# FueledByRedBull/audio-forge

Measured on AMD Instinct MI355X. Metric: 48 kHz mono frames/s (real-time-factor x streams), voice chain, higher is better.
Workload: dtype f64

## Files before the change

### audio-forge_amd/csrc/af_rnnoise.hip

```cpp
#include <hip/hip_runtime.h>
#include <cstdlib>

#include "af_dsp.h"
#include "af_fft_consts.h"
#include "af_suppressor.h"
#include "af_switches.hpp"

namespace af {

__constant__ int c_eband[kRnnBands] = {0, 1, 2, 3, 4, 5, 6, 7, 8, 10, 12, 14, 16, 20, 24, 28, 34, 40, 48, 60, 78, 100};

__constant__ uint16_t c_blk_first[54] = {0, 4, 8, 12, 16, 20, 24, 28, 32, 40, 48, 56, 64, 72, 80, 88, 96, 104, 112, 120, 128, 136, 144, 152, 160, 168, 176, 184, 192, 200, 208, 216, 224, 232, 240, 248, 256, 264, 272, 280, 288, 296, 304, 312, 320, 328, 336, 344, 352, 360, 368, 376, 384, 392};
__constant__ uint8_t c_blk_count[54] = {4, 4, 4, 4, 4, 4, 4, 4, 8, 8, 8, 8, 8, 8, 8, 8, 8, 8, 8, 8, 8, 8, 8, 8, 8, 8, 8, 8, 8, 8, 8, 8, 8, 8, 8, 8, 8, 8, 8, 8, 8, 8, 8, 8, 8, 8, 8, 8, 8, 8, 8, 8, 8, 8};
__constant__ uint8_t c_seg_blk0[21] = {0, 1, 2, 3, 4, 5, 6, 7, 8, 9, 10, 11, 12, 14, 16, 18, 21, 24, 28, 34, 43};
__constant__ uint8_t c_seg_nblk[21] = {1, 1, 1, 1, 1, 1, 1, 1, 1, 1, 1, 1, 2, 2, 2, 3, 3, 4, 6, 9, 11};
constexpr int kBandBlocks = 54;
constexpr int kFftBuf = 15 * 72;
constexpr int kFftWaves = 4;
#ifndef AF_FFT_PREFETCH
#define AF_FFT_PREFETCH 1
#endif
constexpr int kBandSkewLen = 404 + (404 >> 3) + 1;

__device__ __forceinline__ int band_skew(int bin) { return bin + (bin >> 3); }

struct FftShared {
  float2 tw960[15 * 64];
  float2 tw64[8 * 8];
  float win[kRnnFrame];
  float frac[kBandSkewLen];
  int32_t band_of[484];
  float dct6[kRnnBands * 6];
  uint16_t blk_first[64];
  uint8_t blk_count[64], seg_blk0[32], seg_nblk[32];
};

__device__ __forceinline__ float2 cmul(float2 x, float2 w) { return make_float2(x.x * w.x - x.y * w.y, x.x * w.y + x.y * w.x); }
__device__ __forceinline__ float2 cadd(float2 x, float2 y) { return make_float2(x.x + y.x, x.y + y.y); }
__device__ __forceinline__ float2 csub(float2 x, float2 y) { return make_float2(x.x - y.x, x.y - y.y); }
__device__ __forceinline__ float2 mulmj(float2 z) { return make_float2(z.y, -z.x); }

__device__ __forceinline__ void wave_lds_fence() {
  __asm__ volatile("s_waitcnt lgkmcnt(0)" ::: "memory");
  __builtin_amdgcn_wave_barrier();
}

__device__ __forceinline__ void dft3(float2 x0, float2 x1, float2 x2, float2 &y0, float2 &y1, float2 &y2) {
  const float c = 0.86602540378443864676f;
  const float2 t = cadd(x1, x2), d = csub(x1, x2);
  y0 = cadd(x0, t);
  const float2 m = make_float2(x0.x - 0.5f * t.x, x0.y - 0.5f * t.y);
  const float2 sj = make_float2(d.y * c, -d.x * c);
  y1 = cadd(m, sj);
  y2 = csub(m, sj);
}
__device__ __forceinline__ void dft5(const float2 *x, float2 *y) {
  const float c1 = 0.30901699437494742410f, c2 = -0.80901699437494742410f;
  const float s1 = 0.95105651629515357212f, s2 = 0.58778525229247312917f;
  const float2 t1 = cadd(x[1], x[4]), t2 = cadd(x[2], x[3]), d1 = csub(x[1], x[4]), d2 = csub(x[2], x[3]);
  y[0] = make_float2(x[0].x + t1.x + t2.x, x[0].y + t1.y + t2.y);
  const float2 m1 = make_float2(x[0].x + c1 * t1.x + c2 * t2.x, x[0].y + c1 * t1.y + c2 * t2.y);
  const float2 m2 = make_float2(x[0].x + c2 * t1.x + c1 * t2.x, x[0].y + c2 * t1.y + c1 * t2.y);
  const float2 n1 = mulmj(make_float2(s1 * d1.x + s2 * d2.x, s1 * d1.y + s2 * d2.y));
  const float2 n2 = mulmj(make_float2(s2 * d1.x - s1 * d2.x, s2 * d1.y - s1 * d2.y));
  y[1] = cadd(m1, n1);
  y[4] = csub(m1, n1);
  y[2] = cadd(m2, n2);
  y[3] = csub(m2, n2);
}
__device__ __forceinline__ void dft8(const float2 *v, float2 *V) {
  const float h = 0.70710678118654752440f;
  const float2 a0 = cadd(v[0], v[4]), a1 = csub(v[0], v[4]), a2 = cadd(v[2], v[6]), a3 = mulmj(csub(v[2], v[6]));
  const float2 a4 = cadd(v[1], v[5]), a5 = csub(v[1], v[5]), a6 = cadd(v[3], v[7]), a7 = mulmj(csub(v[3], v[7]));
  const float2 b0 = cadd(a0, a2), b2 = csub(a0, a2), b1 = cadd(a1, a3), b3 = csub(a1, a3);
  const float2 b4 = cadd(a4, a6), b6 = csub(a4, a6), b5 = cadd(a5, a7), b7 = csub(a5, a7);
  const float2 w1 = make_float2((b5.x + b5.y) * h, (b5.y - b5.x) * h);
  const float2 w2 = mulmj(b6);
  const float2 w3 = make_float2((b7.y - b7.x) * h, -(b7.x + b7.y) * h);
  V[0] = cadd(b0, b4);
  V[4] = csub(b0, b4);
  V[1] = cadd(b1, w1);
  V[5] = csub(b1, w1);
  V[2] = cadd(b2, w2);
  V[6] = csub(b2, w2);
  V[3] = cadd(b3, w3);
  V[7] = csub(b3, w3);
}

__device__ __forceinline__ void fft_shared_init(FftShared &S, const SuppTables &tb, int tid, int nthreads) {
  for (int i = tid; i < 15 * 64; i += nthreads) S.tw960[i] = tb.twiddle[(i & 63) * (i >> 6)];
  for (int i = tid; i < 64; i += nthreads) S.tw64[i] = tb.twiddle[15 * (i & 7) * (i >> 3)];
  for (int i = tid; i < kRnnFrame; i += nthreads) S.win[i] = tb.half_window[i];
  for (int i = tid; i < 404; i += nthreads) S.frac[band_skew(i)] = tb.frac[i];
  for (int i = tid; i < 484; i += nthreads) S.band_of[i] = tb.band_of_bin[i];
  for (int i = tid; i < kRnnBands * 6; i += nthreads) S.dct6[i] = tb.dct[(i / 6) * kRnnBands + (i % 6)];
  if (tid < 54) {
    S.blk_first[tid] = c_blk_first[tid];
    S.blk_count[tid] = c_blk_count[tid];
  }
  if (tid < 21) {
    S.seg_blk0[tid] = c_seg_blk0[tid];
    S.seg_nblk[tid] = c_seg_nblk[tid];
  }
}

__device__ __forceinline__ void fft960_wave(float2 *a, const FftShared &S, int lane, float scale) {
  float2 x[15];
#pragma unroll
  for (int n1 = 0; n1 < 15; ++n1) x[n1] = a[64 * n1 + lane];
  wave_lds_fence();
  {
    float2 t[3][5];
#pragma unroll
    for (int nb = 0; nb < 5; ++nb)
      dft3(x[(3 * nb) % 15], x[(5 + 3 * nb) % 15], x[(10 + 3 * nb) % 15], t[0][nb], t[1][nb], t[2][nb]);
#pragma unroll
    for (int ka = 0; ka < 3; ++ka) {
      float2 y[5];
      dft5(t[ka], y);
#pragma unroll
      for (int kb = 0; kb < 5; ++kb) {
        const int k1 = (10 * ka + 6 * kb) % 15;
        a[k1 * 72 + lane] = cmul(y[kb], S.tw960[k1 * 64 + lane]);
      }
      __builtin_amdgcn_sched_barrier(0);
    }
  }
  wave_lds_fence();
  {
    const int q = lane & 7;
#pragma unroll
    for (int half = 0; half < 2; ++half) {
      const int id = lane + 64 * half, k1 = id >> 3;
      if (id < 120) {
        float2 v[8], V[8];
#pragma unroll
        for (int pp = 0; pp < 8; ++pp) v[pp] = a[k1 * 72 + 8 * pp + q];
        wave_lds_fence();
        dft8(v, V);
        a[k1 * 72 + q] = V[0];
#pragma unroll
        for (int r = 1; r < 8; ++r) a[k1 * 72 + r * 9 + q] = cmul(V[r], S.tw64[r * 8 + q]);
      }
      __builtin_amdgcn_sched_barrier(0);
    }
  }
  wave_lds_fence();
  {
    float2 v0[8], v1[8];
    const int id1 = lane + 64;
    const int k1a = lane >> 3, r = lane & 7, k1b = id1 >> 3;
#pragma unroll
    for (int q = 0; q < 8; ++q) v0[q] = a[k1a * 72 + r * 9 + q];
    if (id1 < 120) {
#pragma unroll
      for (int q = 0; q < 8; ++q) v1[q] = a[k1b * 72 + r * 9 + q];
    }
    wave_lds_fence();
    float2 V[8];
    dft8(v0, V);
#pragma unroll
    for (int t = 0; t < 8; ++t) a[k1a + 15 * (r + 8 * t)] = make_float2(V[t].x * scale, V[t].y * scale);
    if (id1 < 120) {
      dft8(v1, V);
#pragma unroll
      for (int t = 0; t < 8; ++t) a[k1b + 15 * (r + 8 * t)] = make_float2(V[t].x * scale, V[t].y * scale);
    }
  }
  wave_lds_fence();
}

template <int kBegin, int kEnd, typename F>
__device__ __forceinline__ void static_for(F &&f) {
  if constexpr (kBegin < kEnd) {
    f(std::integral_constant<int, kBegin>{});
    static_for<kBegin + 1, kEnd>(f);
  }
}
template <int kCtrl>
__device__ __forceinline__ float dpp_move(float v) {
  return __int_as_float(__builtin_amdgcn_update_dpp(__float_as_int(v), __float_as_int(v), kCtrl, 0xf, 0xf, false));
}
__device__ __forceinline__ float wave_allsum_xor(float acc) {
  {
    const auto r = __builtin_amdgcn_permlane32_swap(__float_as_uint(acc), __float_as_uint(acc), false, false);
    acc = __uint_as_float(r[0]) + __uint_as_float(r[1]);
  }
  {
    const auto r = __builtin_amdgcn_permlane16_swap(__float_as_uint(acc), __float_as_uint(acc), false, false);
    acc = __uint_as_float(r[0]) + __uint_as_float(r[1]);
  }
  acc = acc + dpp_move<0x128>(acc);
  acc = acc + dpp_move<0x124>(acc);
  acc = acc + dpp_move<0x4E>(acc);
  acc = acc + dpp_move<0xB1>(acc);
  return acc;
}
template <int kN>
__device__ __forceinline__ float wave_dot64_n(const float *x, const float *y, int lane) {
  float acc = 0.0f;
  const float *xl = x + lane, *yl = y + lane;
#pragma unroll
  for (int k = 0; k < (kN + 63) / 64; ++k) {
    if (64 * k + 63 < kN) acc = acc + xl[64 * k] * yl[64 * k];
    else if (lane < kN - 64 * k) acc = acc + xl[64 * k] * yl[64 * k];
  }
  return wave_allsum_xor(acc);
}
__device__ __forceinline__ float wave_dot64_sq_stride2(const float *y, int n, int lane) {
  float acc = 0.0f;
  for (int i = lane; i < n; i += 64) acc = acc + y[2 * i] * y[2 * i];
  return wave_allsum_xor(acc);
}

__device__ __forceinline__ float band_sums_wave(const float *prod, float *scratch, const FftShared &S, int lane) {
  wave_lds_fence();
  float rise = 0.0f, fall = 0.0f;
  if (lane < kBandBlocks) {
    const int e0 = S.blk_first[lane], count = S.blk_count[lane];
#pragma unroll
    for (int j = 0; j < 8; ++j) {
      if (j < count) {
        const int idx = band_skew(e0 + j);
        const float tmp = prod[idx];
        const float fr = S.frac[idx];
        fall += (1 - fr) * tmp;
        rise += fr * tmp;
      }
    }
  }
  scratch[lane] = rise;
  scratch[64 + lane] = fall;
  wave_lds_fence();
  float band = 0.0f;
  if (lane < kRnnBands) {
    float r = 0.0f, f = 0.0f;
    if (lane > 0) {
      const int k0 = S.seg_blk0[lane - 1], nk = S.seg_nblk[lane - 1];
      for (int k = 0; k < nk; ++k) r += scratch[k0 + k];
    }
    if (lane < kRnnBands - 1) {
      const int k0 = S.seg_blk0[lane], nk = S.seg_nblk[lane];
      for (int k = 0; k < nk; ++k) f += scratch[64 + k0 + k];
    }
    band = r + f;
    if (lane == 0 || lane == kRnnBands - 1) band *= 2;
  }
  wave_lds_fence();
  return band;
}

__device__ __forceinline__ float interp_gain(const float *bandE, const FftShared &S, int bin) {
  if (bin >= (100 << 2)) return 0.0f;
  const int b = S.band_of[bin];
  const float f = S.frac[band_skew(bin)];
  return (1 - f) * bandE[b] + f * bandE[b + 1];
}

struct FftUnitLds {
  float2 fa[kFftBuf];
  __device__ float *prod() { return reinterpret_cast<float *>(fa + kRnnFreq + 1); }
  __device__ float *scratch() { return prod() + kBandSkewLen + 1; }
  __device__ float *small() { return scratch() + 128; }
};
static_assert((kRnnFreq + 1) * 2 + kBandSkewLen + 1 + 128 + 6 * 32 <= kFftBuf * 2, "the tail of the transform buffer holds the band work arrays");


constexpr int kFramesPerWave = 10;

__device__ __forceinline__ float window_at(const FftShared &S, int i) { return S.win[i < kRnnFrame ? i : kRnnWindow - 1 - i]; }

extern "C" __global__ __launch_bounds__(64 * kFftWaves, 3) void supp_spectrum_kernel(SuppArgs a, SuppTables tb) {
  __shared__ FftShared S;
  __shared__ FftUnitLds U[kFftWaves];
  const int tid = threadIdx.x, wave = tid >> 6, lane = tid & 63;
  fft_shared_init(S, tb, tid, 64 * kFftWaves);
  __syncthreads();
  const int groups = (a.n_frames + kFramesPerWave - 1) / kFramesPerWave;
  const int64_t unit = (int64_t)blockIdx.x * kFftWaves + wave;
  if (unit >= (int64_t)a.n_streams * groups) return;
  const int s = (int)(unit / groups), fg = (int)(unit % groups);
  const int64_t n = (int64_t)a.n_frames * kRnnFrame;
  FftUnitLds &L = U[wave];
  float nxt[15];
  auto fetch = [&](int f) {
    const float *pb = a.xh + (int64_t)s * (kPitchBuf + n) + (int64_t)(f + 1) * kRnnFrame;
#pragma unroll
    for (int j = 0; j < 15; ++j) nxt[j] = pb[kPitchBuf - kRnnWindow + lane + 64 * j];
  };
  const int f_end = (fg + 1) * kFramesPerWave < a.n_frames ? (fg + 1) * kFramesPerWave : a.n_frames;
  fetch(fg * kFramesPerWave);
  for (int f = fg * kFramesPerWave; f < f_end; ++f) {
    const int64_t cell = (int64_t)f * a.n_streams + s;
#pragma unroll
    for (int j = 0; j < 15; ++j) L.fa[lane + 64 * j] = make_float2(nxt[j] * window_at(S, lane + 64 * j), 0.0f);
#if AF_FFT_PREFETCH
    if (f + 1 < f_end) fetch(f + 1);
#endif
    wave_lds_fence();
    fft960_wave(L.fa, S, lane, 1.0f / kRnnWindow);
#if !AF_FFT_PREFETCH
    if (f + 1 < f_end) fetch(f + 1);
#endif
    float2 *Xg = a.X + cell * kRnnFreq;
    float *prod = L.prod();
#pragma unroll
    for (int j = 0; j < 8; ++j) {
      const int i = lane + 64 * j;
      if (i < kRnnFreq) {
        const float2 x = L.fa[i];
        Xg[i] = x;
        if (i < 400) prod[band_skew(i)] = x.x * x.x + x.y * x.y;
      }
    }
    const float ex = band_sums_wave(prod, L.scratch(), S, lane);
    if (lane < kRnnBands) a.rec[cell].Ex[lane] = ex;
  }
}

struct PitchLds {
  float ds[kPitchBuf / 2];
  float ylk[(kPitchMax >> 1) + 4];
  float ceps[kCepsMem][kRnnBands];
  float Ex[kRnnBands], Ly[kRnnBands];
  float feat[kRnnFeatPad];
  float dist[kCepsMem][kCepsMem];
};

template <int MP>
__device__ __forceinline__ void best_pitch_scan_wave(const float *numa, const float *da, float *syy, float Syy, int lane, int &bp0, int &bp1) {
#pragma unroll 8
  for (int i = 0; i < MP; ++i) {
    syy[i] = Syy;
    Syy = fmaxf(1.0f, Syy + da[i]);
  }
  wave_lds_fence();
  float bn0 = -1, bn1 = -1, bd0 = 0, bd1 = 0;
  bp0 = 0;
  bp1 = 1;
#pragma unroll
  for (int base = 0; base < MP; base += 64) {
    const int i = base + lane;
    const float num = i < MP ? numa[i] : -1.0f;
    const float sy = i < MP ? syy[i] : 1.0f;
    unsigned long long todo = ~0ull;
    for (;;) {
      const bool pass = num >= 0.0f && num * bd1 > bn1 * sy;
      const unsigned long long m = __ballot(pass) & todo;
      if (m == 0) break;
      const int k = __ffsll((long long)m) - 1;
      const float nk = __int_as_float(__builtin_amdgcn_readlane(__float_as_int(num), k));
      const float sk = __int_as_float(__builtin_amdgcn_readlane(__float_as_int(sy), k));
      if (nk * bd0 > bn0 * sk) {
        bn1 = bn0; bd1 = bd0; bp1 = bp0;
        bn0 = nk; bd0 = sk; bp0 = base + k;
      } else {
        bn1 = nk; bd1 = sk; bp1 = base + k;
      }
      todo = k == 63 ? 0ull : ~0ull << (k + 1);
    }
  }
}

constexpr int kPsFrames = 4;
constexpr int kPsX0 = 255;
constexpr int kPsRaw = kPitchBuf + (kPsFrames - 1) * kRnnFrame;
struct PsScan {
  union {
    struct { float d4[kPitchBuf / 4]; float numa[152], da[152], syy[152]; float x4z[672]; } c;
    struct { float xc[304], numa[304], da[304], syy[304]; } f;
  };
};
struct alignas(16) PitchSearch4Lds {
  float ds[kPsFrames][kPitchBuf / 2];
  union {
    float raw[kPsRaw];
    PsScan scan[kPsFrames];
  };
};
#ifdef AF_PS_PROFILE
#define AF_PS_DECL long long ps_t[9]; ps_t[8] = clock64()
#define AF_PS_STAMP(k) ps_t[k] = clock64()
#define AF_PS_PRINT                                                                                                        \
  if (lane == 0 && wave == 0 && (blockIdx.x == 0 || blockIdx.x == gridDim.x / 2))                                          \
  printf("pitch search wg %u: span %lld | decimate %lld | autocorr+lpc %lld | whiten+store %lld | coarse xcorr %lld | coarse scan %lld | " \
         "fine xcorr %lld | fine scan %lld | total %lld cycles\n", blockIdx.x, ps_t[0] - ps_t[8], ps_t[1] - ps_t[0], ps_t[2] - ps_t[1],     \
         ps_t[3] - ps_t[2], ps_t[4] - ps_t[3], ps_t[5] - ps_t[4], ps_t[6] - ps_t[5], ps_t[7] - ps_t[6], ps_t[7] - ps_t[8])
#else
#define AF_PS_DECL
#define AF_PS_STAMP(k)
#define AF_PS_PRINT
#endif
extern "C" __global__ __launch_bounds__(64 * kPsFrames, 4) void supp_pitchsearch4_kernel(SuppArgs a, SuppTables tb) {
  __shared__ PitchSearch4Lds L;
  AF_PS_DECL;
  const int tid = threadIdx.x, wave = tid >> 6, lane = tid & 63;
  const int groups = (a.n_frames + kPsFrames - 1) / kPsFrames;
  const int s = (int)(blockIdx.x / groups), f0 = (int)(blockIdx.x % groups) * kPsFrames;
  const int f = f0 + wave;
  const bool live = f < a.n_frames;
  const int64_t n = (int64_t)a.n_frames * kRnnFrame;
  const float *xh = a.xh + (int64_t)s * (kPitchBuf + n);
  {
    const int frames_here = (a.n_frames - f0) < kPsFrames ? (a.n_frames - f0) : kPsFrames;
    const int span = kPitchBuf + (frames_here - 1) * kRnnFrame;
    const float4 *src = reinterpret_cast<const float4 *>(xh + (int64_t)(f0 + 1) * kRnnFrame);
    float4 *dst = reinterpret_cast<float4 *>(L.raw);
    for (int i = tid; i < span / 4; i += 64 * kPsFrames) dst[i] = src[i];
  }
  __syncthreads();
  AF_PS_STAMP(0);
  float *ds = L.ds[wave];
  if (live) {
    const float *pb = L.raw + wave * kRnnFrame;
    static_for<0, (kPitchBuf / 2 + 63) / 64>([&](auto r_tag) {
      constexpr int r = decltype(r_tag)::value;
      const int i = lane + 64 * r;
      if (64 * r + 63 < kPitchBuf / 2 || lane < kPitchBuf / 2 - 64 * r) {
        if (r == 0) ds[i] = i == 0 ? .5f * (.5f * pb[1] + pb[0]) : .5f * (.5f * (pb[2 * i - 1] + pb[2 * i + 1]) + pb[2 * i]);
        else ds[i] = .5f * (.5f * (pb[2 * i - 1] + pb[2 * i + 1]) + pb[2 * i]);
      }
    });
  }
  __syncthreads();
  if (!live) return;
  AF_PS_STAMP(1);
  PsScan &S = L.scan[wave];
  const int64_t cell = (int64_t)f * a.n_streams + s;
  SuppFrameRec *rec = a.rec + cell;
  float n0, n1, n2, n3, n4;
  {
    float ac[5];
    static_for<0, 5>([&](auto k_tag) {
      constexpr int k = decltype(k_tag)::value;
      ac[k] = wave_dot64_n<kPitchBuf / 2 - k>(ds + k, ds, lane);
    });
    ac[0] *= 1.0001f;
    for (int i = 1; i <= 4; ++i) ac[i] -= ac[i] * (.008f * i) * (.008f * i);
    float lpc[4] = {0, 0, 0, 0};
    float error = ac[0];
    if (ac[0] != 0) {
      for (int i = 0; i < 4; ++i) {
        float rr = 0;
        for (int j = 0; j < i; ++j) rr += lpc[j] * ac[i - j];
        rr += ac[i + 1];
        const float r = -rr / error;
        lpc[i] = r;
        for (int j = 0; j < (i + 1) >> 1; ++j) {
          const float t1 = lpc[j], t2 = lpc[i - 1 - j];
          lpc[j] = t1 + r * t2;
          lpc[i - 1 - j] = t2 + r * t1;
        }
        error = error - r * r * error;
        if (error < .001f * ac[0]) break;
      }
    }
    float tmp = 1.0f;
    for (int i = 0; i < 4; ++i) {
      tmp = .9f * tmp;
      lpc[i] = lpc[i] * tmp;
    }
    const float c1 = .8f;
    n0 = lpc[0] + .8f;
    n1 = lpc[1] + c1 * lpc[0];
    n2 = lpc[2] + c1 * lpc[1];
    n3 = lpc[3] + c1 * lpc[2];
    n4 = c1 * lpc[3];
  }
  AF_PS_STAMP(2);
  {
    constexpr int kRounds = (kPitchBuf / 2 + 63) / 64;
    float yv[kRounds];
    static_for<0, kRounds>([&](auto r_tag) {
      constexpr int r = decltype(r_tag)::value;
      const int i = lane + 64 * r;
      float sum = 0.0f;
      if (64 * r + 63 < kPitchBuf / 2 || lane < kPitchBuf / 2 - 64 * r) {
        sum = ds[i];
        if (r == 0) {
          sum += n0 * (i >= 1 ? ds[i >= 1 ? i - 1 : 0] : 0.0f);
          sum += n1 * (i >= 2 ? ds[i >= 2 ? i - 2 : 0] : 0.0f);
          sum += n2 * (i >= 3 ? ds[i >= 3 ? i - 3 : 0] : 0.0f);
          sum += n3 * (i >= 4 ? ds[i >= 4 ? i - 4 : 0] : 0.0f);
          sum += n4 * (i >= 5 ? ds[i >= 5 ? i - 5 : 0] : 0.0f);
        } else {
          sum += n0 * ds[i - 1];
          sum += n1 * ds[i - 2];
          sum += n2 * ds[i - 3];
          sum += n3 * ds[i - 4];
          sum += n4 * ds[i - 5];
        }
      }
      yv[r] = sum;
    });
    wave_lds_fence();
    float *dsg = a.ds + cell * (kPitchBuf / 2);
    static_for<0, kRounds>([&](auto r_tag) {
      constexpr int r = decltype(r_tag)::value;
      const int i = lane + 64 * r;
      if (64 * r + 63 < kPitchBuf / 2 || lane < kPitchBuf / 2 - 64 * r) {
        ds[i] = yv[r];
        dsg[i] = yv[r];
      }
    });
  }
  wave_lds_fence();
  AF_PS_STAMP(3);
  const int max_pitch = kPitchMax - 3 * kPitchMin;
  const float *x_lp = ds + (kPitchMax >> 1);
  int best0, best1;
  {
    constexpr int len = kRnnWindow >> 2, mp = (kPitchMax - 3 * kPitchMin) >> 2;
    static_assert(kPsX0 + (len - 1) + ((len - 1) >> 4) < 672 && 3 + 4 * 95 + 23 + kPsX0 < 672, "x4z holds the data and both guards");
    for (int i = lane; i < kPsX0; i += 64) S.c.x4z[i] = 0.0f;
    for (int i = kPsX0 + len + ((len - 1) >> 4) + lane; i < 672; i += 64) S.c.x4z[i] = 0.0f;
    for (int i = lane; i < kPitchBuf / 4; i += 64) {
      const float v = ds[2 * i];
      S.c.d4[i] = v;
      const int j = i - (kPitchMax >> 2);
      if (j >= 0 && j < len) S.c.x4z[kPsX0 + j + (j >> 4)] = v;
    }
    wave_lds_fence();
    {
      typedef float v4f_ps __attribute__((ext_vector_type(4)));
      v4f_ps acc = {0.0f, 0.0f, 0.0f, 0.0f};
      const int col = lane & 15, kq = lane >> 4;
      const float *ap = S.c.d4 + kq + col;
      const float *bp = S.c.x4z + kPsX0 + kq - 17 * col;
#pragma unroll
      for (int st = 0; st < 96; ++st) {
        const float av = ap[4 * st];
        const float bv = bp[4 * st + (st >> 2)];
        acc = __builtin_amdgcn_mfma_f32_16x16x4f32(av, bv, acc, 0, 0, 0);
      }
#pragma unroll
      for (int r = 0; r < 4; ++r) {
        const int lag = 16 * col + kq * 4 + r;
        if (lag < mp) {
          const float sum = acc[r];
          const float x16 = sum * 1e-12f;
          S.c.numa[lag] = sum > 0 ? x16 * x16 : -1.0f;
          const float ya = S.c.d4[lag + len], yb = S.c.d4[lag];
          S.c.da[lag] = ya * ya - yb * yb;
        }
      }
    }
    AF_PS_STAMP(4);
    float Syy0;
    {
      float acc = 0.0f;
      for (int i = lane; i < len; i += 64) acc = acc + S.c.d4[i] * S.c.d4[i];
      Syy0 = 1.0f + wave_allsum_xor(acc);
    }
    wave_lds_fence();
    static_assert(mp == 147, "coarse lag count");
    best_pitch_scan_wave<mp>(S.c.numa, S.c.da, S.c.syy, Syy0, lane, best0, best1);
  }
  AF_PS_STAMP(5);
  wave_lds_fence();
  {
    constexpr int len = kRnnWindow >> 1, mp = (kPitchMax - 3 * kPitchMin) >> 1;
    for (int i = lane; i < mp; i += 64) {
      S.f.xc[i] = 0.0f;
      S.f.numa[i] = -1.0f;
      const float ya = ds[i + len], yb = ds[i];
      S.f.da[i] = ya * ya - yb * yb;
    }
    wave_lds_fence();
    for (int c = 0; c < 2; ++c) {
      const int centre = 2 * (c == 0 ? best0 : best1);
      for (int i = centre - 2; i <= centre + 2; ++i) {
        if (i < 0 || i >= mp) continue;
        if (c == 1) {
          const int d0 = i - 2 * best0;
          if (d0 <= 2 && d0 >= -2) continue;
        }
        const float v = fmaxf(-1.0f, wave_dot64_n<len>(x_lp, ds + i, lane));
        if (lane == 0) {
          S.f.xc[i] = v;
          const float x16 = v * 1e-12f;
          S.f.numa[i] = v > 0 ? x16 * x16 : -1.0f;
        }
      }
    }
    AF_PS_STAMP(6);
    const float Syy0 = 1.0f + wave_dot64_n<len>(ds, ds, lane);
    wave_lds_fence();
    best_pitch_scan_wave<mp>(S.f.numa, S.f.da, S.f.syy, Syy0, lane, best0, best1);
  }
  int pitch_index;
  {
    int offset = 0;
    if (best0 > 0 && best0 < (max_pitch >> 1) - 1) {
      const float pa = S.f.xc[best0 - 1], pbv = S.f.xc[best0], pc = S.f.xc[best0 + 1];
      if ((pc - pa) > .7f * (pbv - pa)) offset = 1;
      else if ((pa - pc) > .7f * (pbv - pc)) offset = -1;
    }
    pitch_index = kPitchMax - (2 * best0 - offset);
  }
  if (lane == 0) rec->pitch_index = pitch_index;
  AF_PS_STAMP(7);
  AF_PS_PRINT;
}

extern "C" __global__ __launch_bounds__(64, 6) void supp_pitch_kernel(SuppArgs a, SuppTables tb) {
  __shared__ PitchLds L;
  const int lane = threadIdx.x;
  const int s = blockIdx.x;
  const int64_t n = (int64_t)a.n_frames * kRnnFrame;
  const float *xh = a.xh + (int64_t)s * (kPitchBuf + n);
  float *st = a.state + (int64_t)s * SuppState::kCount;
  int last_period = (int)st[SuppState::kLastPeriod];
  float last_gain = st[SuppState::kLastGain];
  int memid = (int)st[SuppState::kMemId];
  for (int i = lane; i < kCepsMem * kRnnBands; i += 64) (&L.ceps[0][0])[i] = st[SuppState::kCeps + i];
  __syncthreads();

  constexpr int kDsRegs = (kPitchBuf / 2 + 63) / 64;
  float ds_next[kDsRegs];
  float ex_next = 0.0f;
  int pitch_next = 0;
  auto prefetch = [&](int f) {
    const SuppFrameRec *rn = a.rec + ((int64_t)f * a.n_streams + s);
    const float *dsg = a.ds + ((int64_t)f * a.n_streams + s) * (kPitchBuf / 2);
#pragma unroll
    for (int k2 = 0; k2 < kDsRegs; ++k2) {
      const int i = lane + 64 * k2;
      ds_next[k2] = i < kPitchBuf / 2 ? dsg[i] : 0.0f;
    }
    ex_next = lane < kRnnBands ? rn->Ex[lane] : 0.0f;
    pitch_next = rn->pitch_index;
  };
  if (a.n_frames > 0) prefetch(0);
  for (int f = 0; f < a.n_frames; ++f) {
    SuppFrameRec *rec = a.rec + ((int64_t)f * a.n_streams + s);
    if (lane < kRnnBands) L.Ex[lane] = ex_next;
#pragma unroll
    for (int k2 = 0; k2 < kDsRegs; ++k2) {
      const int i = lane + 64 * k2;
      if (i < kPitchBuf / 2) L.ds[i] = ds_next[k2];
    }
    int pitch_index = __builtin_amdgcn_readfirstlane(pitch_next);
    const float ex_mine = ex_next;
    if (f + 1 < a.n_frames) prefetch(f + 1);
    __syncthreads();
    float gain;
    {
      const int minperiod0 = kPitchMin;
      const int maxperiod = kPitchMax / 2, minperiod = kPitchMin / 2, N = kRnnWindow / 2;
      int T0 = pitch_index / 2;
      const int prev_period = last_period / 2;
      const float *x = L.ds + maxperiod;
      if (T0 >= maxperiod) T0 = maxperiod - 1;
      const float xx = wave_dot64_n<N>(x, x, lane);
      float xy = wave_dot64_n<N>(x, x - T0, lane);
      {
        const int chunk = (maxperiod + 63) / 64;
        float local[6];
        float acc = 0.0f;
#pragma unroll
        for (int k2 = 0; k2 < 6; ++k2) {
          const int i = lane * chunk + k2 + 1;
          if (i <= maxperiod) acc = acc + (x[-i] * x[-i] - x[N - i] * x[N - i]);
          local[k2] = acc;
        }
        float total = acc;
#pragma unroll
        for (int off = 1; off < 64; off <<= 1) {
          const float other = __shfl_up(total, off);
          if (lane >= off) total = total + other;
        }
        const float before = __shfl_up(total, 1);
        if (lane == 0) L.ylk[0] = xx;
#pragma unroll
        for (int k2 = 0; k2 < 6; ++k2) {
          const int i = lane * chunk + k2 + 1;
          if (i <= maxperiod) L.ylk[i] = fmaxf(0.0f, xx + (lane == 0 ? local[k2] : before + local[k2]));
        }
      }
      __syncthreads();
      float yy = L.ylk[T0];
      float best_xy = xy, best_yy = yy;
      const float g0 = xy / sqrtf(1 + xx * yy);
      float g = g0;
      int T = T0;
      float xy_k[16], yy_k[16];
      int T1_k[16];
      static_for<2, 16>([&](auto k_tag) {
        constexpr int k2 = decltype(k_tag)::value;
        const int T1 = (2 * T0 + k2) / (2 * k2);
        int T1b;
        if (k2 == 2) T1b = (T1 + T0 > maxperiod) ? T0 : T0 + T1;
        else {
          constexpr int sc2 = (k2 == 6 || k2 == 12) ? 5 : ((k2 & 1) ? 2 : 3);
          T1b = (2 * sc2 * T0 + k2) / (2 * k2);
        }
        T1_k[k2] = T1;
        if (T1 >= minperiod) {
          xy_k[k2] = __int_as_float(__builtin_amdgcn_readfirstlane(
              __float_as_int(.5f * (wave_dot64_n<N>(x, x - T1, lane) + wave_dot64_n<N>(x, x - T1b, lane)))));
          yy_k[k2] = __int_as_float(__builtin_amdgcn_readfirstlane(__float_as_int(.5f * (L.ylk[T1] + L.ylk[T1b]))));
        } else {
          xy_k[k2] = 0.0f;
          yy_k[k2] = 0.0f;
        }
        if (k2 & 1) __builtin_amdgcn_sched_barrier(0);
      });
      bool past_min = false;
      static_for<2, 16>([&](auto k_tag) {
        constexpr int k2 = decltype(k_tag)::value;
        const int T1 = T1_k[k2];
        if (T1 < minperiod) past_min = true;
        if (past_min) return;
        xy = xy_k[k2];
        yy = yy_k[k2];
        const float g1 = xy / sqrtf(1 + xx * yy);
        float cont;
        const int dT = T1 - prev_period;
        if (dT <= 1 && dT >= -1) cont = last_gain;
        else if (dT <= 2 && dT >= -2 && 5 * k2 * k2 < T0) cont = .5f * last_gain;
        else cont = 0;
        float thresh = fmaxf(.3f, .7f * g0 - cont);
        if (T1 < 3 * minperiod) thresh = fmaxf(.4f, .85f * g0 - cont);
        else if (T1 < 2 * minperiod) thresh = fmaxf(.5f, .9f * g0 - cont);
        if (g1 > thresh) {
          best_xy = xy;
          best_yy = yy;
          T = T1;
          g = g1;
        }
      });
      best_xy = fmaxf(0.0f, best_xy);
      float pg = (best_yy <= best_xy) ? 1.0f : best_xy / (best_yy + 1);
      const float c0 = wave_dot64_n<N>(x, x - (T - 1), lane);
      const float c1v = wave_dot64_n<N>(x, x - T, lane);
      const float c2 = wave_dot64_n<N>(x, x - (T + 1), lane);
      int offset = 0;
      if ((c2 - c0) > .7f * (c1v - c0)) offset = 1;
      else if ((c0 - c2) > .7f * (c1v - c2)) offset = -1;
      if (pg > g) pg = g;
      pitch_index = 2 * T + offset;
      if (pitch_index < minperiod0) pitch_index = minperiod0;
      gain = pg;
    }
    last_period = pitch_index;
    last_gain = gain;
    float dctcol[kRnnBands];
    {
      int col = lane < kRnnBands ? lane : 0;
      asm volatile("" : "+v"(col));
#pragma unroll
      for (int j = 0; j < kRnnBands; ++j) dctcol[j] = tb.dct[j * kRnnBands + col];
    }
    float E = 0.0f;
    {
      const float ly_raw = log10f(1e-2f + ex_mine);
      float logMax = -2, follow = -2, ly_mine = 0.0f;
#pragma unroll
      for (int i = 0; i < kRnnBands; ++i) {
        float ly = __int_as_float(__builtin_amdgcn_readlane(__float_as_int(ly_raw), i));
        ly = fmaxf(logMax - 7, fmaxf(follow - 1.5f, ly));
        if (lane == i) ly_mine = ly;
        logMax = fmaxf(logMax, ly);
        follow = fmaxf(follow - 1.5f, ly);
        E += __int_as_float(__builtin_amdgcn_readlane(__float_as_int(ex_mine), i));
      }
      if (lane < kRnnBands) L.Ly[lane] = ly_mine;
    }
    const bool silence = E < 0.04f;
    if (lane < kRnnFeatPad) L.feat[lane] = 0.0f;
    __syncthreads();
    if (!silence) {
      if (lane == 6) L.feat[kRnnBands + 18] = .01f * (pitch_index - 300);
      if (lane < kRnnBands) {
        float sum = 0;
#pragma unroll
        for (int j = 0; j < kRnnBands; ++j) sum += L.Ly[j] * dctcol[j];
        float v = sum * sqrtf(2.0f / 22);
        if (lane == 0) v -= 12;
        if (lane == 1) v -= 4;
        L.feat[lane] = v;
        L.ceps[memid][lane] = v;
      }
      __syncthreads();
      const int m1 = memid < 1 ? kCepsMem + memid - 1 : memid - 1;
      const int m2 = memid < 2 ? kCepsMem + memid - 2 : memid - 2;
      if (lane < 6) {
        const float c0 = L.ceps[memid][lane], c1v = L.ceps[m1][lane], c2 = L.ceps[m2][lane];
        L.feat[lane] = c0 + c1v + c2;
        L.feat[kRnnBands + lane] = c0 - c2;
        L.feat[kRnnBands + 6 + lane] = c0 - 2 * c1v + c2;
      }
      memid = memid + 1 == kCepsMem ? 0 : memid + 1;
      {
        const int i = lane >> 3, j = lane & 7;
        float dist = 0;
        for (int k2 = 0; k2 < kRnnBands; ++k2) {
          const float t = L.ceps[i][k2] - L.ceps[j][k2];
          dist += t * t;
        }
        L.dist[i][j] = dist;
      }
      __syncthreads();
      {
        float mindist = 1e15f;
        if (lane < kCepsMem) {
#pragma unroll
          for (int j = 0; j < kCepsMem; ++j)
            if (j != lane) mindist = fminf(mindist, L.dist[lane][j]);
        }
        float spec_variability = 0;
#pragma unroll
        for (int i = 0; i < kCepsMem; ++i) spec_variability += __int_as_float(__builtin_amdgcn_readlane(__float_as_int(mindist), i));
        if (lane == 0) L.feat[kRnnBands + 19] = spec_variability / kCepsMem - 2.1f;
      }
    }
    __syncthreads();
    if (lane < kRnnFeatPad) rec->feat[lane] = L.feat[lane];
    if (lane == 0) {
      rec->silence = silence ? 1 : 0;
      rec->pitch_index = pitch_index;
    }
    __syncthreads();
  }
  if (lane == 0) {
    st[SuppState::kLastPeriod] = (float)last_period;
    st[SuppState::kLastGain] = last_gain;
    st[SuppState::kMemId] = (float)memid;
  }
  for (int i = lane; i < kCepsMem * kRnnBands; i += 64) st[SuppState::kCeps + i] = (&L.ceps[0][0])[i];
  for (int i = lane; i < kPitchBuf; i += 64) st[SuppState::kHist + i] = xh[n + i];
}

extern "C" __global__ __launch_bounds__(64 * kFftWaves, 3) void supp_pitchspec_kernel(SuppArgs a, SuppTables tb) {
  __shared__ FftShared S;
  __shared__ FftUnitLds U[kFftWaves];
  const int tid = threadIdx.x, wave = tid >> 6, lane = tid & 63;
  fft_shared_init(S, tb, tid, 64 * kFftWaves);
  __syncthreads();
  const int groups = (a.n_frames + kFramesPerWave - 1) / kFramesPerWave;
  const int64_t unit = (int64_t)blockIdx.x * kFftWaves + wave;
  if (unit >= (int64_t)a.n_streams * groups) return;
  const int s = (int)(unit / groups), fg = (int)(unit % groups);
  const int64_t n = (int64_t)a.n_frames * kRnnFrame;
  FftUnitLds &L = U[wave];
  const int f_begin = fg * kFramesPerWave;
  const int f_end = (fg + 1) * kFramesPerWave < a.n_frames ? (fg + 1) * kFramesPerWave : a.n_frames;
  int my_pitch = 0, my_silence = 0;
  if (f_begin + lane < f_end) {
    const SuppFrameRec *r = a.rec + ((int64_t)(f_begin + lane) * a.n_streams + s);
    my_pitch = r->pitch_index;
    my_silence = r->silence;
  }
  float nxt[15];
  auto fetch = [&](int f) {
    const int pitch_index = __builtin_amdgcn_readlane(my_pitch, f - f_begin);
    const float *pb = a.xh + (int64_t)s * (kPitchBuf + n) + (int64_t)(f + 1) * kRnnFrame;
#pragma unroll
    for (int j = 0; j < 15; ++j) nxt[j] = pb[kPitchBuf - kRnnWindow - pitch_index + lane + 64 * j];
  };
  fetch(f_begin);
  for (int f = f_begin; f < f_end; ++f) {
    const int64_t cell = (int64_t)f * a.n_streams + s;
    SuppFrameRec *rec = a.rec + cell;
    const bool silence = __builtin_amdgcn_readlane(my_silence, f - f_begin) != 0;
    const float2 *Xg = a.X + cell * kRnnFreq;
    float2 Xr[8];
#pragma unroll
    for (int j = 0; j < 8; ++j) {
      const int i = lane + 64 * j;
      Xr[j] = i < kRnnFreq ? Xg[i] : make_float2(0.0f, 0.0f);
    }
    float ex = 0.0f;
    if (lane < kRnnBands) ex = rec->Ex[lane];
#pragma unroll
    for (int j = 0; j < 15; ++j) L.fa[lane + 64 * j] = make_float2(nxt[j] * window_at(S, lane + 64 * j), 0.0f);
#if AF_FFT_PREFETCH
    if (f + 1 < f_end) fetch(f + 1);
#endif
    wave_lds_fence();
    fft960_wave(L.fa, S, lane, 1.0f / kRnnWindow);
#if !AF_FFT_PREFETCH
    if (f + 1 < f_end) fetch(f + 1);
#endif
    float2 *Pg = a.P + cell * kRnnFreq;
    float *prod = L.prod();
    float2 Pr[7];
#pragma unroll
    for (int j = 0; j < 8; ++j) {
      const int i = lane + 64 * j;
      if (i < kRnnFreq) {
        const float2 p = L.fa[i];
        Pg[i] = p;
        if (j < 7) Pr[j] = p;
        if (i < 400) prod[band_skew(i)] = p.x * p.x + p.y * p.y;
      }
    }
// ... 569 lines not shown
```

Measured before the change: 13.02 billion.

## Shrink coarse pitch MFMA to ten rows and scan fine candidates in registers

The coarse cross-correlation MFMA now runs 64 steps over a 10-row lag map instead of 96 steps over a padded layout, using a new index-map header with different LDS padding. The fine pitch search no longer fills and scans a full 304-lag array. It keeps the up to ten candidate correlations in lanes, computes the running Syy prefix only up to the highest candidate, and picks the best two with a ballot-based scan. This cuts LDS traffic and serial scan work, at the cost of more intricate index logic that must reproduce the original tie-breaking and Syy accumulation exactly.

```diff
diff --git a/audio-forge_amd/csrc/af_pitch_coarse_map.h b/audio-forge_amd/csrc/af_pitch_coarse_map.h
--- /dev/null
+++ b/audio-forge_amd/csrc/af_pitch_coarse_map.h
@@ -0,0 +1,39 @@
+#pragma once
+
+namespace af {
+namespace pitch_coarse {
+
+constexpr int kSteps = 64;
+constexpr int kLen = 240;
+constexpr int kLags = 147;
+constexpr int kRows = 10;
+constexpr int kYLen = 432;
+constexpr int kXGuardLo = 15;
+constexpr int kXGuardHi = 16;
+constexpr int kXWords = kXGuardLo + kLen + kXGuardHi;
+
+constexpr int y_word(int m) { return m + (m >> 4); }
+constexpr int kYWords = y_word(kYLen - 1) + 1;
+
+constexpr int lane_row(int lane) { return lane & 15; }
+constexpr int lane_k(int lane) { return lane >> 4; }
+constexpr int used_row(int row) { return row < kRows ? row : kRows - 1; }
+
+constexpr int y_index(int step, int k, int row) { return 4 * step + k + 16 * used_row(row); }
+constexpr int x_index(int step, int k, int col) { return 4 * step + k - col; }
+
+constexpr int a_base(int k, int row) { return 17 * used_row(row) + k; }
+constexpr int a_step(int step) { return 4 * step + (step >> 2); }
+constexpr int a_word(int step, int k, int row) { return a_base(k, row) + a_step(step); }
+constexpr int b_base(int k, int col) { return kXGuardLo + k - col; }
+constexpr int b_step(int step) { return 4 * step; }
+constexpr int b_word(int step, int k, int col) { return b_base(k, col) + b_step(step); }
+
+constexpr int out_row(int lane, int r) { return 4 * (lane >> 4) + r; }
+constexpr int out_lag(int lane, int r) { return 16 * out_row(lane, r) + (lane & 15); }
+
+static_assert(a_word(kSteps - 1, 3, kRows - 1) == y_word(4 * (kSteps - 1) + 3 + 16 * (kRows - 1)), "the padded word of the largest y index");
+static_assert(a_word(kSteps - 1, 3, 15) < kYWords && b_word(kSteps - 1, 3, 0) == kXWords - 1 && b_word(0, 0, 15) == 0, "operand ranges");
+
+}
+}
diff --git a/audio-forge_amd/csrc/af_rnnoise.hip b/audio-forge_amd/csrc/af_rnnoise.hip
--- a/audio-forge_amd/csrc/af_rnnoise.hip
+++ b/audio-forge_amd/csrc/af_rnnoise.hip
@@ -3,6 +3,7 @@
 
 #include "af_dsp.h"
 #include "af_fft_consts.h"
+#include "af_pitch_coarse_map.h"
 #include "af_suppressor.h"
 #include "af_switches.hpp"
 
@@ -362,15 +363,38 @@
   }
 }
 
+__device__ __forceinline__ void best_pitch_scan_candidates(float num, float sy, int lag, int &bp0, int &bp1) {
+  float bn0 = -1, bn1 = -1, bd0 = 0, bd1 = 0;
+  bp0 = 0;
+  bp1 = 1;
+  unsigned long long todo = ~0ull;
+  for (;;) {
+    const bool pass = num >= 0.0f && num * bd1 > bn1 * sy;
+    const unsigned long long m = __ballot(pass) & todo;
+    if (m == 0) break;
+    const int k = __ffsll((long long)m) - 1;
+    const float nk = __int_as_float(__builtin_amdgcn_readlane(__float_as_int(num), k));
+    const float sk = __int_as_float(__builtin_amdgcn_readlane(__float_as_int(sy), k));
+    const int pk = __builtin_amdgcn_readlane(lag, k);
+    if (nk * bd0 > bn0 * sk) {
+      bn1 = bn0; bd1 = bd0; bp1 = bp0;
+      bn0 = nk; bd0 = sk; bp0 = pk;
+    } else {
+      bn1 = nk; bd1 = sk; bp1 = pk;
+    }
+    todo = k == 63 ? 0ull : ~0ull << (k + 1);
+  }
+}
+
 constexpr int kPsFrames = 4;
-constexpr int kPsX0 = 255;
 constexpr int kPsRaw = kPitchBuf + (kPsFrames - 1) * kRnnFrame;
 struct PsScan {
   union {
-    struct { float d4[kPitchBuf / 4]; float numa[152], da[152], syy[152]; float x4z[672]; } c;
-    struct { float xc[304], numa[304], da[304], syy[304]; } f;
+    struct { float y4p[460]; float xz[272]; float numa[152], da[152], syy[152]; } c;
+    struct { float da[304]; } f;
   };
 };
+static_assert(pitch_coarse::kYWords <= 460 && pitch_coarse::kXWords <= 272 && pitch_coarse::kYLen == kPitchBuf / 4, "coarse operands");
 struct alignas(16) PitchSearch4Lds {
   float ds[kPsFrames][kPitchBuf / 2];
   union {
@@ -510,37 +534,37 @@
   const float *x_lp = ds + (kPitchMax >> 1);
   int best0, best1;
   {
+    namespace cm = pitch_coarse;
     constexpr int len = kRnnWindow >> 2, mp = (kPitchMax - 3 * kPitchMin) >> 2;
-    static_assert(kPsX0 + (len - 1) + ((len - 1) >> 4) < 672 && 3 + 4 * 95 + 23 + kPsX0 < 672, "x4z holds the data and both guards");
-    for (int i = lane; i < kPsX0; i += 64) S.c.x4z[i] = 0.0f;
-    for (int i = kPsX0 + len + ((len - 1) >> 4) + lane; i < 672; i += 64) S.c.x4z[i] = 0.0f;
+    static_assert(len == cm::kLen && mp == cm::kLags && (kPitchMax >> 2) + len == cm::kYLen, "the map's shape");
+    if (lane < cm::kXGuardLo) S.c.xz[lane] = 0.0f;
+    if (lane < cm::kXGuardHi) S.c.xz[cm::kXGuardLo + len + lane] = 0.0f;
     for (int i = lane; i < kPitchBuf / 4; i += 64) {
       const float v = ds[2 * i];
-      S.c.d4[i] = v;
+      S.c.y4p[cm::y_word(i)] = v;
       const int j = i - (kPitchMax >> 2);
-      if (j >= 0 && j < len) S.c.x4z[kPsX0 + j + (j >> 4)] = v;
+      if (j >= 0) S.c.xz[cm::kXGuardLo + j] = v;
     }
     wave_lds_fence();
     {
       typedef float v4f_ps __attribute__((ext_vector_type(4)));
       v4f_ps acc = {0.0f, 0.0f, 0.0f, 0.0f};
-      const int col = lane & 15, kq = lane >> 4;
-      const float *ap = S.c.d4 + kq + col;
-      const float *bp = S.c.x4z + kPsX0 + kq - 17 * col;
-#pragma unroll
-      for (int st = 0; st < 96; ++st) {
-        const float av = ap[4 * st];
-        const float bv = bp[4 * st + (st >> 2)];
+      const float *ap = S.c.y4p + cm::a_base(cm::lane_k(lane), cm::lane_row(lane));
+      const float *bp = S.c.xz + cm::b_base(cm::lane_k(lane), cm::lane_row(lane));
+#pragma unroll
+      for (int st = 0; st < cm::kSteps; ++st) {
+        const float av = ap[cm::a_step(st)];
+        const float bv = bp[cm::b_step(st)];
         acc = __builtin_amdgcn_mfma_f32_16x16x4f32(av, bv, acc, 0, 0, 0);
       }
 #pragma unroll
       for (int r = 0; r < 4; ++r) {
-        const int lag = 16 * col + kq * 4 + r;
-        if (lag < mp) {
+        const int lag = cm::out_lag(lane, r);
+        if (cm::out_row(lane, r) < cm::kRows && lag < mp) {
           const float sum = acc[r];
           const float x16 = sum * 1e-12f;
           S.c.numa[lag] = sum > 0 ? x16 * x16 : -1.0f;
-          const float ya = S.c.d4[lag + len], yb = S.c.d4[lag];
+          const float ya = S.c.y4p[cm::y_word(lag + len)], yb = S.c.y4p[cm::y_word(lag)];
           S.c.da[lag] = ya * ya - yb * yb;
         }
       }
@@ -549,7 +573,10 @@
     float Syy0;
     {
       float acc = 0.0f;
-      for (int i = lane; i < len; i += 64) acc = acc + S.c.d4[i] * S.c.d4[i];
+      for (int i = lane; i < len; i += 64) {
+        const float v = S.c.y4p[cm::y_word(i)];
+        acc = acc + v * v;
+      }
       Syy0 = 1.0f + wave_allsum_xor(acc);
     }
     wave_lds_fence();
@@ -558,41 +585,56 @@
   }
   AF_PS_STAMP(5);
   wave_lds_fence();
+  int lag_l = -1;
+  float xc_l = 0.0f;
   {
     constexpr int len = kRnnWindow >> 1, mp = (kPitchMax - 3 * kPitchMin) >> 1;
-    for (int i = lane; i < mp; i += 64) {
-      S.f.xc[i] = 0.0f;
-      S.f.numa[i] = -1.0f;
+    const int lo = 2 * (best0 < best1 ? best0 : best1), hi = 2 * (best0 < best1 ? best1 : best0);
+    const int last = hi + 2 < mp ? hi + 2 : mp - 1;
+    for (int i = lane; i < last; i += 64) {
       const float ya = ds[i + len], yb = ds[i];
       S.f.da[i] = ya * ya - yb * yb;
     }
+    float num_l = -1.0f, sy_l = 1.0f;
+    for (int q = 0; q < 10; ++q) {
+      const int i = q < 5 ? lo - 2 + q : hi - 7 + q;
+      if (i < 0 || i >= mp || (q >= 5 && i <= lo + 2)) continue;
+      const float v = fmaxf(-1.0f, wave_dot64_n<len>(x_lp, ds + i, lane));
+      if (lane == q) {
+        lag_l = i;
+        xc_l = v;
+        const float x16 = v * 1e-12f;
+        num_l = v > 0 ? x16 * x16 : -1.0f;
+      }
+    }
+    AF_PS_STAMP(6);
+    float Syy = 1.0f + wave_dot64_n<len>(ds, ds, lane);
     wave_lds_fence();
-    for (int c = 0; c < 2; ++c) {
-      const int centre = 2 * (c == 0 ? best0 : best1);
-      for (int i = centre - 2; i <= centre + 2; ++i) {
-        if (i < 0 || i >= mp) continue;
-        if (c == 1) {
-          const int d0 = i - 2 * best0;
-          if (d0 <= 2 && d0 >= -2) continue;
-        }
-        const float v = fmaxf(-1.0f, wave_dot64_n<len>(x_lp, ds + i, lane));
-        if (lane == 0) {
-          S.f.xc[i] = v;
-          const float x16 = v * 1e-12f;
-          S.f.numa[i] = v > 0 ? x16 * x16 : -1.0f;
-        }
-      }
-    }
-    AF_PS_STAMP(6);
-    const float Syy0 = 1.0f + wave_dot64_n<len>(ds, ds, lane);
-    wave_lds_fence();
-    best_pitch_scan_wave<mp>(S.f.numa, S.f.da, S.f.syy, Syy0, lane, best0, best1);
+    int i = 0;
+    for (int g = 0; g < 2; ++g) {
+      const int start = (g == 0 ? lo : hi) - 2;
+#pragma unroll 8
+      for (; i < start; ++i) Syy = fmaxf(1.0f, Syy + S.f.da[i]);
+#pragma unroll
+      for (int q = 0; q < 5; ++q) {
+        const int c = start + q;
+        if (c < i || c >= mp) continue;
+        if (lag_l == c) sy_l = Syy;
+        if (c < last) Syy = fmaxf(1.0f, Syy + S.f.da[c]);
+        i = c + 1;
+      }
+    }
+    best_pitch_scan_candidates(num_l, sy_l, lag_l, best0, best1);
   }
   int pitch_index;
   {
     int offset = 0;
     if (best0 > 0 && best0 < (max_pitch >> 1) - 1) {
-      const float pa = S.f.xc[best0 - 1], pbv = S.f.xc[best0], pc = S.f.xc[best0 + 1];
+      auto xc_at = [&](int i) {
+        const unsigned long long m = __ballot(lag_l == i);
+        return m ? __int_as_float(__builtin_amdgcn_readlane(__float_as_int(xc_l), __ffsll((long long)m) - 1)) : 0.0f;
+      };
+      const float pa = xc_at(best0 - 1), pbv = xc_at(best0), pc = xc_at(best0 + 1);
       if ((pc - pa) > .7f * (pbv - pa)) offset = 1;
       else if ((pa - pc) > .7f * (pbv - pc)) offset = -1;
     }
```

Measured after the change: 13.39 billion, median of 6. 1.03x the previous value.
